# ming71/rotate-yolov3

Hardware: AMD Instinct MI355X
Metric: images/sec fwd+bwd at 608^2 (train step, backend=hip) (higher is better)
Workload: dtype bf16; 1 GPU; configs[3]: Darknet-53 train step (fwd + riou loss + bwd + grad all-reduce + SGD), bs=64/GPU 608x608, synthetic HRSC-shaped targets; global_batch=64, parallelism=dp1, gradients=250 MB fp32 in 4 flat buckets, fp32 on the wire

## Files before the change

include/ryolo.h:

```cpp
#ifndef RYOLO_H
#define RYOLO_H

#include <stddef.h>
#include <stdint.h>

#ifdef __cplusplus
extern "C" {
#endif

#define RYOLO_OK 0
#define RYOLO_EINVAL -1
#define RYOLO_ELAUNCH -2
#define RYOLO_ETOOBIG -3

#define RYOLO_RNMS_MAX_BOXES 262144

const char *ryolo_strerror(int code);
int ryolo_abi_version(void);
const char *ryolo_build_id(void);
int ryolo_set_tuning(const char *name, const char *value);

size_t ryolo_rnms_workspace_bytes(int n);
int ryolo_rnms(const float *dets, int n, int row_stride, float thr, int64_t *keep_out, int32_t *num_keep,
               void *workspace, size_t workspace_bytes, void *stream);
// ... 190 lines not shown
#define RYOLO_ARC_UBCE 2
#define RYOLO_ARC_UCE 4
size_t ryolo_yolo_loss_bitmap_bytes_arc(long long cells, int nc, int arc);
int ryolo_yolo_loss_arc(const float *p, int bs, int na, int ny, int nx, int no, int nc, const float *w, int NT,
                        const long long *b, const long long *gj, const long long *gi, const long long *cls, const float *txy,
                        const float *twh, const float *ta, const float *anchor_vec, const float *npos, float giou, float reg_w,
                        float cls_w, float cls_pw, float obj_w, float obj_pw, int iou_mode, int arc, float fl_gamma, unsigned *bitmap,
                        float *dp, float *items, void *stream);
int ryolo_yolo_loss_nhwc_arc(const void *head, int head_cstride, const float *p, int bs, int na, int ny, int nx, int no, int nc,
                             const float *w, int NT, const long long *b, const long long *gj, const long long *gi,
                             const long long *cls, const float *txy, const float *twh, const float *ta, const float *anchor_vec,
                             const float *npos, float giou, float reg_w, float cls_w, float cls_pw, float obj_w, float obj_pw,
                             int iou_mode, int arc, float fl_gamma, unsigned *bitmap, float *dp_sparse, void *head_grad,
                             int head_grad_cstride, float *items, void *stream);
int ryolo_scale_bf16_if(const float *g, void *buf, int cstride, long long npix, int C, void *stream);

int ryolo_riou_loss_pairs(const float *pbox, const float *tbox, int n, float *iou, float *grad, void *stream);

typedef struct ryolo_sgd_job {
    void *p;
    const void *g;
    void *buf;
    long long n;
    int group, first, block_begin, block_end;
} ryolo_sgd_job;
int ryolo_sgd_step(const ryolo_sgd_job *device_jobs, int njobs, int total_blocks, const float *group_hparams, int nesterov,
                   void *stream);

#ifdef __cplusplus
}
// ... 3 lines not shown
```

rotate-yolov3_amd/csrc/loss.hip:

```cpp
#include <hip/hip_runtime.h>
#include <stdint.h>

#include "../../include/ryolo.h"
#include "riou_grad.h"

namespace {

__device__ __forceinline__ float softplusf(float x) { return fmaxf(x, 0.f) + log1pf(__expf(-fabsf(x))); }
__device__ __forceinline__ float sigmoidf(float x) { return 1.f / (1.f + __expf(-x)); }
__device__ __forceinline__ float sl1(float d) { const float a = fabsf(d); return a < 1.f ? 0.5f * d * d : a - 0.5f; }
__device__ __forceinline__ float sl1_grad(float d) { return fabsf(d) < 1.f ? d : (d > 0.f ? 1.f : -1.f); }

struct Focal { float fl, f; };
__device__ __forceinline__ Focal focal_of(float L, float gamma, bool on) {
    if (!on) return Focal{L, 1.f};
    const float e = expf(-L), q = 1.000001f - e, m = powf(q, gamma);
    return Focal{L * m, m + L * gamma * (m / q) * e};
}

__device__ __forceinline__ float wave_sum(float v) {
#pragma unroll
    for (int o = 32; o > 0; o >>= 1) v += __shfl_xor(v, o);
    return v;
}
// ... 172 lines not shown
                }
            }
        }
    }
    l_obj = wave_sum(l_obj);
    l_cls = wave_sum(l_cls);
    l_reg = wave_sum(l_reg);
    if ((threadIdx.x & 63) == 0) {
        if (l_obj != 0.f) atomicAdd(q.items + 0, l_obj);
        if (l_cls != 0.f) atomicAdd(q.items + 1, l_cls);
        if (l_reg != 0.f) atomicAdd(q.items + 2, l_reg);
    }
}

typedef __attribute__((ext_vector_type(8))) __bf16 loss_bf16x8;
template <int NO>
__global__ void __launch_bounds__(256)
yolo_loss_dense_nhwc_kernel(const __bf16 *__restrict__ head, int head_cs, long long npix, int plane, int na, int no_rt, float coef,
                            float *__restrict__ dp, const unsigned *__restrict__ bitmap, __bf16 *__restrict__ hg, int hg_cs,
                            float *__restrict__ items) {
    const int no = NO ? NO : no_rt;
    const int cpr = na * no / 8;
    float acc = 0.f;
    const int lane = threadIdx.x & 63;
    const long long wave0 = (long long)blockIdx.x * 4 + (threadIdx.x >> 6), nwaves = (long long)gridDim.x * 4;
    auto one = [&](long long pix, int c8, const loss_bf16x8 &v) {
        const int a0 = c8 / no, k0 = c8 - a0 * no;
        int e1 = 5 - k0;
        if (e1 < 0) e1 += no;
        const int e2 = e1 + no;
        const uint4 raw = __builtin_bit_cast(uint4, v);
        auto logit = [&](int e) {
            const int w = e >> 1;
            unsigned d = raw.x;
            d = w == 1 ? raw.y : d;
            d = w == 2 ? raw.z : d;
            d = w == 3 ? raw.w : d;
            return __builtin_bit_cast(float, (e & 1) ? (d & 0xffff0000u) : (d << 16));
        };
        auto objectness = [&](float x) {
            const float ex = __expf(-fabsf(x));
            const float r = __builtin_amdgcn_rcpf(1.f + ex);
            acc += fmaxf(x, 0.f) + __logf(1.f + ex);
            return coef * (x >= 0.f ? r : ex * r);
        };
        float g1 = 0.f, g2 = 0.f;
        if (e1 < 8) g1 = objectness(logit(e1));
        if (e2 < 8) g2 = objectness(logit(e2));
        auto place = [&](float g, int e, unsigned (&ow)[4]) {
            const unsigned bits = (unsigned)__builtin_bit_cast(unsigned short, (__bf16)g) << ((e & 1) * 16);
#pragma unroll
            for (int w = 0; w < 4; w++) ow[w] |= (e >> 1) == w ? bits : 0u;
        };
        unsigned ow[4] = {0u, 0u, 0u, 0u};
        if (e1 < 8) place(g1, e1, ow);
        if (e2 < 8) place(g2, e2, ow);
        const long long bit0 = pix * na + a0;
        const int nspan = (k0 + 7) / no;
        unsigned hits = 0;
        for (int j = 0; j <= nspan; j++) hits |= ((bitmap[(bit0 + j) >> 5] >> ((bit0 + j) & 31)) & 1u) << j;
        if (hits) {
            const unsigned n = (unsigned)pix / (unsigned)plane;
            const long long cell0 = ((long long)n * na) * plane + ((unsigned)pix - n * (unsigned)plane);
            int j = 0, k = k0;
#pragma unroll
            for (int e = 0; e < 8; e++) {
                float o = (e == e1 ? g1 : 0.f) + (e == e2 ? g2 : 0.f);
                if ((hits >> j) & 1u) {
                    float *src = dp + (cell0 + (long long)(a0 + j) * plane) * no + k;
                    o += *src;
                    *src = 0.f;
                }
                const unsigned bits = (unsigned)__builtin_bit_cast(unsigned short, (__bf16)o);
                ow[e >> 1] = (e & 1) ? (ow[e >> 1] & 0xffffu) | (bits << 16) : (ow[e >> 1] & 0xffff0000u) | bits;
                if (++k == no) {
                    k = 0;
                    j++;
                }
            }
        }
        *(uint4 *)(hg + pix * hg_cs + c8) = uint4{ow[0], ow[1], ow[2], ow[3]};
    };
    for (long long pix = wave0; pix < npix; pix += nwaves)
        for (int chunk = lane; chunk < cpr; chunk += 64) one(pix, chunk * 8, *(const loss_bf16x8 *)(head + pix * head_cs + chunk * 8));
    __shared__ float wsum[4];
    acc = wave_sum(acc);
    if ((threadIdx.x & 63) == 0) wsum[threadIdx.x >> 6] = acc;
    __syncthreads();
    if (threadIdx.x == 0) {
        const float t = (wsum[0] + wsum[1]) + (wsum[2] + wsum[3]);
        if (t != 0.f) atomicAdd(items + 0, t * coef);
    }
}

__global__ void __launch_bounds__(256)
yolo_loss_dense_arc_kernel(const __bf16 *__restrict__ head, int head_cs, const float *__restrict__ p, long long cells, long long npix,
                           int plane, int na, int no, int nc, int focal, int unified, float gamma, float coef, float *__restrict__ dp,
                           const unsigned *__restrict__ bitmap, __bf16 *__restrict__ hg, int hg_cs, float *__restrict__ items) {
    float acc = 0.f;
    for (long long i = (long long)blockIdx.x * blockDim.x + threadIdx.x; i < cells; i += (long long)gridDim.x * blockDim.x) {
        float x[32], g[32];
        long long cell;
        long long pix = 0;
        int a = 0;
        if (head) {
            pix = i / na;
            a = (int)(i - pix * na);
// ... 52 lines not shown
__global__ void scale_bf16_if_kernel(const float *__restrict__ g, __bf16 *__restrict__ buf, int cs, long long npix, int C) {
    const float sc = g[0];
    if (sc == 1.f) return;
    const int cpr = C / 8;
    const long long total = npix * cpr;
    for (long long i = (long long)blockIdx.x * blockDim.x + threadIdx.x; i < total; i += (long long)gridDim.x * blockDim.x) {
        const long long pix = i / cpr;
        const int c8 = (int)(i - pix * cpr) * 8;
        loss_bf16x8 v = *(loss_bf16x8 *)(buf + pix * cs + c8);
#pragma unroll
        for (int e = 0; e < 8; e++) v[e] = (__bf16)((float)v[e] * sc);
        *(loss_bf16x8 *)(buf + pix * cs + c8) = v;
    }
}

struct BuildTargetsParams {
    const float *tpad;
    const unsigned char *valid;
    int NT, nheads, na;
    float iou_t, ang_t, cf;
    const float *ng[RYOLO_MAX_HEADS];
    const float *av[RYOLO_MAX_HEADS];
    float *w[RYOLO_MAX_HEADS];
    long long *idx[RYOLO_MAX_HEADS];
    float *box[RYOLO_MAX_HEADS];
    float *npos[RYOLO_MAX_HEADS];
};

__global__ void __launch_bounds__(256) build_targets_kernel(const BuildTargetsParams q) {
    const int t = blockIdx.x * blockDim.x + threadIdx.x;
// ... 153 lines not shown
                         const long long *cls, const float *txy, const float *twh, const float *ta, const float *anchor_vec,
                         const float *npos, float giou, float reg_w, float cls_w, float cls_pw, float obj_w, float obj_pw,
                         int iou_mode, unsigned *bitmap, float *dp_sparse, void *head_grad, int head_grad_cstride, float *items,
                         void *stream_) {
    return ryolo_yolo_loss_nhwc_arc(head, head_cstride, p, bs, na, ny, nx, no, nc, w, NT, b, gj, gi, cls, txy, twh, ta, anchor_vec, npos,
                                    giou, reg_w, cls_w, cls_pw, obj_w, obj_pw, iou_mode, 0, 0.f, bitmap, dp_sparse, head_grad,
                                    head_grad_cstride, items, stream_);
}

int ryolo_yolo_loss_nhwc_arc(const void *head, int head_cstride, const float *p, int bs, int na, int ny, int nx, int no, int nc,
                             const float *w, int NT, const long long *b, const long long *gj, const long long *gi,
                             const long long *cls, const float *txy, const float *twh, const float *ta, const float *anchor_vec,
                             const float *npos, float giou, float reg_w, float cls_w, float cls_pw, float obj_w, float obj_pw,
                             int iou_mode, int arc, float fl_gamma, unsigned *bitmap, float *dp_sparse, void *head_grad,
                             int head_grad_cstride, float *items, void *stream_) {
    if (!arc_ok(arc, no, nc)) return RYOLO_EINVAL;
    if (!head || !p || !w || !b || !gj || !gi || !cls || !txy || !twh || !ta || !anchor_vec || !npos || !bitmap || !dp_sparse ||
        !head_grad || !items)
        return RYOLO_EINVAL;
    if (bs <= 0 || na <= 0 || ny <= 0 || nx <= 0 || no < 6 + (nc > 1 ? nc : 0) || NT <= 0 || (iou_mode != 0 && iou_mode != 1))
        return RYOLO_EINVAL;
    const int C = na * no;
    if ((C & 7) || (head_cstride & 7) || (head_grad_cstride & 7) || head_cstride < C || head_grad_cstride < C ||
        ((uintptr_t)head & 15) || ((uintptr_t)head_grad & 15))
        return RYOLO_EINVAL;
    hipStream_t stream = (hipStream_t)stream_;
    const long long cells = (long long)bs * na * ny * nx, npix = (long long)bs * ny * nx;
    const float coef = obj_w / (float)cells;
    const int rc = launch_positives(p, dp_sparse, bs, na, ny, nx, no, nc, w, NT, b, gj, gi, cls, txy, twh, ta, anchor_vec, npos,
                                    giou, reg_w, cls_w, cls_pw, coef, obj_pw, iou_mode, bitmap, items, stream, arc, fl_gamma, 1);
    if (rc != RYOLO_OK) return rc;
    long long nb = (npix * (C / 8) + 255) / 256;
    if (nb > 2048) nb = 2048;
    if (nb < 1) nb = 1;
    if (arc != 0) {
        const int unified = (arc & RYOLO_ARC_UBCE) ? 1 : ((arc & RYOLO_ARC_UCE) ? 2 : 0);
        const float cf = unified == 1 ? coef / (float)(nc > 1 ? nc : 1) : (unified == 2 ? cls_w / (float)cells : coef);
        long long nbc = (cells + 255) / 256;
        if (nbc > 4096) nbc = 4096;
        hipLaunchKernelGGL(yolo_loss_dense_arc_kernel, dim3((unsigned)nbc), dim3(256), 0, stream, (const __bf16 *)head, head_cstride,
                           (const float *)nullptr, cells, npix, ny * nx, na, no, nc, (arc & RYOLO_ARC_FOCAL) ? 1 : 0, unified, fl_gamma,
                           cf, dp_sparse, bitmap, (__bf16 *)head_grad, head_grad_cstride, items);
        return hipGetLastError() == hipSuccess ? RYOLO_OK : RYOLO_ELAUNCH;
    }
    if (npix >= 0x7fffffffll) return RYOLO_EINVAL;
    nb = (npix + 3) / 4;
    if (nb > 8192) nb = 8192;
    if (no == 7)
        hipLaunchKernelGGL(yolo_loss_dense_nhwc_kernel<7>, dim3((unsigned)nb), dim3(256), 0, stream, (const __bf16 *)head,
                           head_cstride, npix, ny * nx, na, no, coef, dp_sparse, bitmap, (__bf16 *)head_grad, head_grad_cstride,
                           items);
    else
        hipLaunchKernelGGL(yolo_loss_dense_nhwc_kernel<0>, dim3((unsigned)nb), dim3(256), 0, stream, (const __bf16 *)head,
                           head_cstride, npix, ny * nx, na, no, coef, dp_sparse, bitmap, (__bf16 *)head_grad, head_grad_cstride,
                           items);
    return hipGetLastError() == hipSuccess ? RYOLO_OK : RYOLO_ELAUNCH;
}

int ryolo_scale_bf16_if(const float *g, void *buf, int cstride, long long npix, int C, void *stream) {
    if (!g || !buf || npix <= 0 || C <= 0 || (C & 7) || (cstride & 7) || cstride < C) return RYOLO_EINVAL;
    long long nb = (npix * (C / 8) + 255) / 256;
    if (nb > 2048) nb = 2048;
    hipLaunchKernelGGL(scale_bf16_if_kernel, dim3((unsigned)nb), dim3(256), 0, (hipStream_t)stream, g, (__bf16 *)buf, cstride, npix, C);
    return hipGetLastError() == hipSuccess ? RYOLO_OK : RYOLO_ELAUNCH;
}

int ryolo_yolo_loss(const float *p, int bs, int na, int ny, int nx, int no, int nc, const float *w, int NT,
                    const long long *b, const long long *gj, const long long *gi, const long long *cls, const float *txy,
                    const float *twh, const float *ta, const float *anchor_vec, const float *npos, float giou, float reg_w,
                    float cls_w, float cls_pw, float obj_w, float obj_pw, int iou_mode, unsigned *bitmap, float *dp,
// ... 40 lines not shown
```

rotate-yolov3_amd/model/hip_train_ops.py:

```python
import ctypes as C

import torch

from .. import _lib
from .hip_ops import ConvDesc, _check_nhwc, cpad

_vp = C.c_void_p
_P = C.POINTER(ConvDesc)
_lib.declare("ryolo_conv_stat_rows", C.c_int, [_P])
_lib.declare("ryolo_conv2d_bn_act_stats", C.c_int, [_P, _vp, _vp, _vp, _vp, _vp, _vp, _vp, _vp])
_lib.declare("ryolo_bn_finalize", C.c_int, [_vp, C.c_int, C.c_int, C.c_int, C.c_longlong, C.c_float, C.c_float, _vp, _vp, _vp,
                                            _vp, _vp, _vp, _vp, _vp, _vp])
_lib.declare("ryolo_bn_act_fwd", C.c_int, [_vp, C.c_int, _vp, _vp, C.c_int, _vp, _vp, C.c_int, _vp, C.c_int, C.c_longlong,
                                           C.c_int, _vp])
_lib.declare("ryolo_bn_act_bwd_workspace_bytes", C.c_size_t, [C.c_longlong, C.c_int])
_lib.declare("ryolo_bn_act_bwd", C.c_int, [_vp, C.c_int, _vp, C.c_int, _vp, _vp, _vp, _vp, C.c_int, _vp, _vp, C.c_int,
                                           C.c_longlong, C.c_int, _vp, _vp, _vp, _vp, C.c_size_t, _vp])
_lib.declare("ryolo_conv_packed_dgrad_bytes", C.c_size_t, [C.c_int, C.c_int, C.c_int, C.c_int])
_lib.declare("ryolo_conv_pack_weights_dgrad", C.c_int, [_vp, C.c_int, C.c_int, C.c_int, C.c_int, _vp, _vp, _vp])
_lib.declare("ryolo_conv_dgrad_tap_table", C.c_int, [C.c_int, C.c_int, _vp])
_lib.declare("ryolo_conv2d_dgrad", C.c_int, [_P, _vp, C.c_int, _vp, _vp, _vp, _vp, C.c_int, _vp])
_lib.declare("ryolo_conv2d_dgrad_bnreduce", C.c_int, [_P, _vp, C.c_int, _vp, _vp, _vp, _vp, C.c_int, _vp, C.c_int, _vp, _vp, _vp, _vp, _vp,
                                                      _vp, _vp])
_lib.declare("ryolo_bn_act_bwd_reduced", C.c_int, [_vp, C.c_int, _vp, C.c_int, _vp, _vp, _vp, _vp, C.c_int, _vp, _vp, C.c_int,
# ... 7 lines not shown


_lib.declare("ryolo_yolo_loss_bitmap_bytes", C.c_size_t, [C.c_longlong])
_lib.declare("ryolo_yolo_loss", C.c_int, [_vp, C.c_int, C.c_int, C.c_int, C.c_int, C.c_int, C.c_int, _vp, C.c_int, _vp, _vp, _vp,
                                          _vp, _vp, _vp, _vp, _vp, _vp, C.c_float, C.c_float, C.c_float, C.c_float, C.c_float,
                                          C.c_float, C.c_int, _vp, _vp, _vp, _vp])
_lib.declare("ryolo_yolo_loss_nhwc", C.c_int, [_vp, C.c_int, _vp, C.c_int, C.c_int, C.c_int, C.c_int, C.c_int, C.c_int, _vp, C.c_int, _vp,
                                               _vp, _vp, _vp, _vp, _vp, _vp, _vp, _vp, C.c_float, C.c_float, C.c_float, C.c_float,
                                               C.c_float, C.c_float, C.c_int, _vp, _vp, _vp, C.c_int, _vp, _vp])
_lib.declare("ryolo_scale_bf16_if", C.c_int, [_vp, _vp, C.c_int, C.c_longlong, C.c_int, _vp])
_lib.declare("ryolo_yolo_loss_bitmap_bytes_arc", C.c_size_t, [C.c_longlong, C.c_int, C.c_int])
_lib.declare("ryolo_yolo_loss_arc", C.c_int, [_vp] + [C.c_int] * 6 + [_vp, C.c_int] + [_vp] * 9 + [C.c_float] * 6 +
             [C.c_int, C.c_int, C.c_float] + [_vp] * 4)
_lib.declare("ryolo_yolo_loss_nhwc_arc", C.c_int, [_vp, C.c_int, _vp] + [C.c_int] * 6 + [_vp, C.c_int] + [_vp] * 9 + [C.c_float] * 6 +
             [C.c_int, C.c_int, C.c_float] + [_vp, _vp, _vp, C.c_int, _vp, _vp])
ARC_FOCAL, ARC_UBCE, ARC_UCE = 1, 2, 4


def arc_flags(arc):
    f = ARC_FOCAL if 'F' in arc else 0
    if 'default' in arc:
        return f
    if 'BCE' in arc:
        return f | ARC_UBCE
    if 'CE' in arc:
        return f | ARC_UCE
    raise ValueError("unknown arc %r" % (arc,))
_lib.declare("ryolo_riou_loss_pairs", C.c_int, [_vp, _vp, C.c_int, _vp, _vp, _vp])


# ... 312 lines not shown
    bs, na, ny, nx, no = p.shape
    w = hd['w'].contiguous()
    n = hd['npos'] if 'npos' in hd else w.sum()
    c = lambda t: t.contiguous()
    b, gj, gi, cls = c(hd['b']), c(hd['gj']), c(hd['gi']), c(hd['cls'])
    txy, twh, ta, av = c(hd['gxy']), c(hd['gwh']), c(hd['ga']), c(hd['av'].float())
    _lib.check(_lib.lib().ryolo_yolo_loss_arc(p.data_ptr(), bs, na, ny, nx, no, nc, w.data_ptr(), w.shape[1], b.data_ptr(),
                                              gj.data_ptr(), gi.data_ptr(), cls.data_ptr(), txy.data_ptr(), twh.data_ptr(),
                                              ta.data_ptr(), av.data_ptr(), n.data_ptr(), float(h['giou']), float(h['reg']),
                                              float(h['cls']), float(h['cls_pw']), float(h['obj']), float(h['obj_pw']),
                                              1 if h.get('riou', 0) else 0, int(arc), float(h.get('fl_gamma', 0.0)),
                                              bitmap.data_ptr(), dp.data_ptr(), items.data_ptr(), _s(p.device)),
               "ryolo_yolo_loss_arc")


def yolo_loss_head_nhwc(head, p, hd, nc, h, bitmap, dp_sparse, head_g, items, arc=0):
    bs, na, ny, nx, no = p.shape
    w = hd['w'].contiguous()
    n = hd['npos'] if 'npos' in hd else w.sum()
    c = lambda t: t.contiguous()
    b, gj, gi, cls = c(hd['b']), c(hd['gj']), c(hd['gi']), c(hd['cls'])
    txy, twh, ta, av = c(hd['gxy']), c(hd['gwh']), c(hd['ga']), c(hd['av'].float())
    _lib.check(_lib.lib().ryolo_yolo_loss_nhwc_arc(head.data_ptr(), head.stride(2), p.data_ptr(), bs, na, ny, nx, no, nc, w.data_ptr(),
                                                   w.shape[1], b.data_ptr(), gj.data_ptr(), gi.data_ptr(), cls.data_ptr(),
                                                   txy.data_ptr(), twh.data_ptr(), ta.data_ptr(), av.data_ptr(), n.data_ptr(),
                                                   float(h['giou']), float(h['reg']), float(h['cls']), float(h['cls_pw']),
                                                   float(h['obj']), float(h['obj_pw']), 1 if h.get('riou', 0) else 0, int(arc),
                                                   float(h.get('fl_gamma', 0.0)), bitmap.data_ptr(), dp_sparse.data_ptr(),
                                                   head_g.data_ptr(), head_g.stride(2), items.data_ptr(), _s(p.device)),
               "ryolo_yolo_loss_nhwc_arc")


def scale_bf16_if(g, buf):
    n, hh, ww, cc = buf.shape
    _lib.check(_lib.lib().ryolo_scale_bf16_if(g.data_ptr(), buf.data_ptr(), buf.stride(2), n * hh * ww, cc, _s(buf.device)),
               "ryolo_scale_bf16_if")


class RotatedIoU(torch.autograd.Function):

    @staticmethod
    def forward(ctx, pbox, tbox):
        if not pbox.is_cuda:
            raise RuntimeError("RotatedIoU runs on the HIP kernel only (got a CPU tensor)")
        p = pbox.detach().float().contiguous()
        t = tbox.detach().float().contiguous()
        n = p.shape[0]
        iou = torch.empty(n, dtype=torch.float32, device=p.device)
        grad = torch.empty(n, 5, dtype=torch.float32, device=p.device)
        _lib.check(_lib.lib().ryolo_riou_loss_pairs(p.data_ptr(), t.data_ptr(), n, iou.data_ptr(), grad.data_ptr(), _s(p.device)),
                   "ryolo_riou_loss_pairs")
# ... 43 lines not shown
```

rotate-yolov3_amd/model/loss_static.py:

```python
import math

import os

import torch
import torch.nn.functional as F

from .loss import _core


def pad_targets(targets, capacity):
    nt = int(targets.shape[0])
    if nt > capacity:
        raise ValueError("pad_targets: %d targets exceed the capacity %d" % (nt, capacity))
    tpad = torch.zeros(capacity, 7, dtype=torch.float32, device=targets.device)
    valid = torch.zeros(capacity, dtype=torch.bool, device=targets.device)
    if nt:
        tpad[:nt] = targets
        valid[:nt] = True
    return tpad, valid


def _smooth_l1(a, b):
    d = (a - b).abs()
    return torch.where(d < 1.0, 0.5 * d * d, d - 0.5)
# ... 109 lines not shown
        return fused.static_loss.clone()

    @staticmethod
    def backward(ctx, g):
        if ctx.stamp != ctx.state['stamp']:
            raise RuntimeError("fused compute_loss: backward() of a loss whose head gradients were overwritten by a later "
                               "compute_loss call on the same engine (call backward before computing the next loss)")
        if ctx.used:
            raise RuntimeError("fused compute_loss: second backward() through the same loss (the head-gradient buffers were "
                               "scaled in place by the first; retain_graph is not supported on the fused path)")
        ctx.used = True
        pg = ctx.fused.pg
        heads = ctx.fused.head_grads
        if heads is not None:
            from . import hip_train_ops as tr
            g1 = g.detach().reshape(1).float()
            for hg in heads:
                tr.scale_bf16_if(g1, hg)
        else:
            for buf in pg:
                buf.mul_(g)
        return (None,) + tuple(pg)


class FusedLoss(object):

    def __init__(self, model, capacity=512, impl='hip'):
        self.model = model
        self.impl = impl
        self.capacity = int(capacity)
        self._last_state = None

    def _engine_of(self, p):
# ... 50 lines not shown
                    eng.graph_fallback = "loss: %s: %s" % (type(e).__name__, str(e).splitlines()[0][:200] if str(e) else "")
                    import warnings
                    warnings.warn("fused loss: hipGraph capture failed (%s); continuing with eager launches" % eng.graph_fallback)
                    try:
                        torch.cuda.synchronize(dev)
                    except Exception:
                        pass
                    self._body(st)
            if st['graph'] is not None:
                st['graph'].replay()
        st['calls'] += 1
        st['stamp'] = st.get('stamp', 0) + 1
        self._last_state = st
        if st.get('head_g') is not None:
            eng.head_g_ready = True
        loss = _FusedLossFn.apply(self, *p)
        return loss, torch.cat((st['items'][:3], loss.detach()))

    def _make_state(self, eng, hyp, key):
        dev = eng.device
        if not hasattr(eng, "static_pg"):
            eng.static_pg = [torch.zeros_like(q) for q in eng.p]
        h = self.model.hyp if getattr(self.model, 'hyp', None) else hyp
        pairs = getattr(eng, 'head_pairs', None)
        nhwc = self.impl == 'hip' and pairs is not None and all(
            (hd.shape[-1] % 8 == 0 and q.shape[1] * q.shape[4] == hd.shape[-1]) for (hd, _), q in zip(pairs, eng.p))
        if nhwc:
            eng.fused_nhwc = True
            for buf in eng.static_pg:
                buf.zero_()
        return dict(key=key, hyp=dict(hyp), calls=0, graph=None, pg=eng.static_pg, eng=eng,
                    head=[a for a, _ in pairs] if nhwc else None, head_g=[b for _, b in pairs] if nhwc else None,
                    leaves=[q.detach().requires_grad_(True) for q in eng.p],
                    t=torch.zeros(self.capacity, 7, device=dev), valid=torch.zeros(self.capacity, dtype=torch.bool, device=dev),
                    loss=torch.zeros(1, device=dev), items=torch.zeros(4, device=dev),
                    pw=(torch.tensor([h['cls_pw']], dtype=torch.float32, device=dev),
                        torch.tensor([h['obj_pw']], dtype=torch.float32, device=dev)))

    def _body(self, st):
        if self.impl == 'hip':
            return self._body_hip(st)
        with torch.enable_grad():
            loss, items = compute_loss_static(st['leaves'], st['t'], st['valid'], self.model, st['hyp'], pos_weights=st['pw'])
            grads = torch.autograd.grad(loss, st['leaves'])
        with torch.no_grad():
            for buf, g in zip(st['pg'], grads):
                buf.copy_(g)
            st['loss'].copy_(loss.detach())
            st['items'].copy_(items)

    def _body_hip(self, st):
        from . import hip_train_ops as tr
        core = self.model
        h = core.hyp if getattr(core, 'hyp', None) else st['hyp']
        with torch.no_grad():
            if 'bt' not in st:
                st['bt'] = tr.BuildTargets(core, self.capacity, st['t'].device)
                st['valid_u8'] = torch.zeros(self.capacity, dtype=torch.uint8, device=st['t'].device)
            st['valid_u8'].copy_(st['valid'])
            st['bt'].run(st['t'], st['valid_u8'], h, st['hyp']['context_factor'])
            heads = st['bt'].heads()
            arc = tr.arc_flags(core.arc)
            if 'bitmaps' not in st:
                st['bitmaps'] = [tr.yolo_loss_bitmap(q, core.nc, arc) for q in st['leaves']]
            st['items'].zero_()
            for k, (q, hd, bm, dp) in enumerate(zip(st['leaves'], heads, st['bitmaps'], st['pg'])):
                bm.zero_()
                if st.get('head_g') is not None:
                    tr.yolo_loss_head_nhwc(st['head'][k], q.detach(), hd, core.nc, h, bm, dp, st['head_g'][k], st['items'], arc)
                else:
                    tr.yolo_loss_head(q.detach(), hd, core.nc, h, bm, dp, st['items'], arc)

            st['items'][3:4].copy_(st['items'][:3].sum(0, keepdim=True))
            st['loss'].copy_(st['items'][3:4])
```

rotate-yolov3_amd/model/train_engine.py:

```python
import ctypes as C
import os

import torch
import torch.nn as nn

from .. import _lib
from . import hip_ops as ops
from . import hip_train_ops as tr
from . import plan
from .engine import HipEngine


class _Fn(torch.autograd.Function):
    @staticmethod
    def forward(ctx, engine, x, anchor):
        ctx.engine = engine
        outs = engine.forward(x)
        return tuple(outs)

    @staticmethod
    def backward(ctx, *grads):
        ctx.engine.backward(grads)
        return None, None, None

# ... 71 lines not shown
            elif kind in ('add', 'up'):
                fwd.append((kind, i, tuple(tv(v) for v in rec)))
            elif kind == 'yolo':
                m = mods[i]
                c, h, w = tp.shapes[i]
                anchors = m.anchors.to(device=device, dtype=torch.float32).contiguous()
                pbuf = torch.empty((self.bs, m.na, h, w, model.nc + 6), dtype=torch.float32, device=device)
                io = None
                if model.nc + 6 > 96 or m.na * (model.nc + 6) > 1024:
                    io = torch.empty((self.bs, m.na * h * w, model.nc + 6), dtype=torch.float32, device=device)
                self.p.append(pbuf)
                fwd.append(('yolo', i, (tv(rec[0]), tv(rec[1]), m, anchors, pbuf, io, h, w)))
        self.head_pairs = [(pl[0], pl[1]) for kind, _, pl in fwd if kind == 'yolo']
        self.fused_nhwc = False
        self.head_g_ready = False
        self.batch_reduce = os.environ.get('RYOLO_WGRAD_BATCH_REDUCE', '1') != '0'
        self._wr_batches = {}
        self._ws_w_bytes = max(wgrad_ws, 256)
        self._ws_w = None
        self.ws_b = torch.empty(max(bn_ws, 256), dtype=torch.uint8, device=device)

        self.bplan = [(kind, i, pl, flags) for (kind, i, pl), (_, _, flags) in zip(reversed(fwd), tp.backward)]

    @staticmethod
    def _conv_attrs(m):
        conv = HipEngine._conv_of(m)
        other = [type(s_).__name__ for s_ in m if not isinstance(s_, (nn.Conv2d, nn.BatchNorm2d, nn.PReLU, nn.LeakyReLU))
                 and type(s_).__name__ != 'Mish']
        return dict(cout=conv.out_channels, k=conv.kernel_size[0], s=conv.stride[0], pad=conv.padding[0],
                    bn=HipEngine._bn_of(m) is not None, act=None,
# ... 248 lines not shown
                stride = float(max(self.H, self.W)) / float(max(hh, ww))
                _lib.check(L.ryolo_yolo_decode(head.data_ptr(), head.stride(2), self.bs, hh, ww, m.na, self.model.nc + 6,
                                               anchors.data_ptr(), stride, 1.0, 0, io.data_ptr() if io is not None else None, m.na * hh * ww, 0,
                                               pbuf.data_ptr(), _lib.stream_ptr(dev)), "ryolo_yolo_decode")
                if (m.nx, m.ny) != (ww, hh):
                    from .models import create_grids
                    create_grids(m, (self.H, self.W), (ww, hh), dev)

    def backward(self, pgrads):
        dev = self.device
        with torch.cuda.device(dev), torch.no_grad():
            if not hasattr(self, "static_pg"):
                self.static_pg = [torch.zeros_like(p) for p in self.p]
            ready = self.head_g_ready
            self.head_g_ready = False
            for k, (buf, g) in enumerate(zip(self.static_pg, pgrads)):
                if g is not None and ready and g.data_ptr() == buf.data_ptr():
                    continue
                if g is None:
                    buf.zero_()
                elif g.data_ptr() != buf.data_ptr():
                    buf.copy_(g)
                tr.pgrad_to_nhwc(buf, self.head_pairs[k][1])
                if self.fused_nhwc and g is not None:
                    buf.zero_()
            self._check_direct_sink()
            self._grad_of(next(self.model.parameters()))
            segs = self._segments()
            if self.batch_reduce:
                self._ensure_reduce_batches(segs)
            if self.g_bwd is None:
                self.g_bwd = [None] * len(segs)
            for k, (lo, hi, params) in enumerate(segs):
                if not self.use_graph or self.steps < 2 or self.force_eager:
                    self._backward_launch(lo, hi)
                else:
                    if self.g_bwd[k] is None:
                        self.g_bwd[k] = self._capture(lambda lo=lo, hi=hi: self._backward_launch(lo, hi))
                    if self.g_bwd[k] is not None:
                        self.g_bwd[k].replay()
                self._flush_param_grads(params)
            self.steps += 1

    def _backward_launch(self, lo=0, hi=None):
        dev = self.device
        L = _lib.lib()
        pgrads = self.static_pg
# ... 22 lines not shown
                                              self._grad_of(bn.weight), self._grad_of(bn.bias), dsl, self._grad_of(conv.weight),
                                              conv.in_channels, True, b['ws0f'])
                        return
                    elif b['recompute']:
                        if 'ws0' not in b:
                            b['ws0'] = tr.conv0_bn_bwd_ws(dev)
                        tr.conv0_bn_bwd(b['desc'], b['xin'], b['packed'], dy, b['stats'], b['actcode'], b['slope'], b['dz'],
                                        self._grad_of(bn.weight), self._grad_of(bn.bias), dsl, b['ws0'])
                    elif b.get('red_part') is not None:
                        tr.bn_act_bwd_reduced(b['z'], dy, b['stats'], 1, b['slope'], b['dz'],
                                              self._grad_of(bn.weight), self._grad_of(bn.bias), dsl, b['red_part'], self.ws_b)
                    else:
                        tr.bn_act_bwd(b['z'], dy, b['stats'], b['actcode'], b['slope'], b['dz'],
                                      self._grad_of(bn.weight), self._grad_of(bn.bias), dsl, self.ws_b)
                elif conv.bias is not None:
                    tr.bn_act_bwd(b['z'], dy, None, 0, None, None, None, self._grad_of(conv.bias), None, self.ws_b)
                if self.batch_reduce:
                    tr.conv_wgrad_partials(b['desc'], b['xin'], b['dz'], conv.in_channels, self._grad_of(conv.weight), True, b['ws_w'])
                else:
                    tr.conv_wgrad(b['desc'], b['xin'], b['dz'], conv.in_channels, self._grad_of(conv.weight), True, self.ws_w)
                if b['xin_g'] is not None:
                    y = b.get('red_for')
                    if y is not None:
                        tr.conv_dgrad_bnreduce(b['desc'], b['dz'], b['packed_d'], self.ones, self.zeros, b['xin_g'], not in_first,
                                               y['z'], y['stats'], y['slope'], y['red_part'])
                    else:
                        tr.conv_dgrad(b['desc'], b['dz'], b['packed_d'], self.ones, self.zeros, b['xin_g'], not in_first)
            elif kind == 'add':
                dyv = pl[5]
                self._passthrough(dyv, pl[3], flags[0])
                self._passthrough(dyv, pl[4], flags[1])
# ... 45 lines not shown
```

Baseline: 1341 images/s.

## Fuse head conv bias-gradient reduction into dense NHWC loss kernel

The dense NHWC YOLO loss kernel can now accumulate per-block partial column sums of the bf16 head gradient into a bias_part buffer. A small two-stage reduction kernel later folds these partials and applies the loss gradient scale to produce the head conv bias gradient, replacing a full bn_act_bwd pass over the head gradient. Separately, the per-head bf16 gradient scaling launches are batched into one multi-head kernel using a persistent device scale tensor. This adds shared-memory accumulation to the loss kernel and a separate graph cache per mode, and relies on the loss scale being linear so scaling after reduction matches.

```diff
diff --git a/include/ryolo.h b/include/ryolo.h
--- a/include/ryolo.h
+++ b/include/ryolo.h
@@ -228,6 +228,18 @@
                              int iou_mode, int arc, float fl_gamma, unsigned *bitmap, float *dp_sparse, void *head_grad,
                              int head_grad_cstride, float *items, void *stream);
 int ryolo_scale_bf16_if(const float *g, void *buf, int cstride, long long npix, int C, void *stream);
+int ryolo_scale_bf16_if_heads(const float *g, void *const *bufs, const int *cstrides, const long long *npixs, const int *Cs, int nheads,
+                              void *stream);
+
+int ryolo_yolo_loss_dbias_rows(int bs, int na, int ny, int nx, int no, int arc);
+size_t ryolo_head_dbias_part_floats(int rows, int C);
+int ryolo_yolo_loss_nhwc_dbias(const void *head, int head_cstride, const float *p, int bs, int na, int ny, int nx, int no, int nc,
+                               const float *w, int NT, const long long *b, const long long *gj, const long long *gi,
+                               const long long *cls, const float *txy, const float *twh, const float *ta, const float *anchor_vec,
+                               const float *npos, float giou, float reg_w, float cls_w, float cls_pw, float obj_w, float obj_pw,
+                               int iou_mode, int arc, float fl_gamma, unsigned *bitmap, float *dp_sparse, void *head_grad,
+                               int head_grad_cstride, float *items, float *bias_part, int bias_part_rows, void *stream);
+int ryolo_head_dbias_finalize(float *part, int rows, int C, const float *scale, float *dbias, void *stream);
 
 int ryolo_riou_loss_pairs(const float *pbox, const float *tbox, int n, float *iou, float *grad, void *stream);
 
diff --git a/rotate-yolov3_amd/csrc/loss.hip b/rotate-yolov3_amd/csrc/loss.hip
--- a/rotate-yolov3_amd/csrc/loss.hip
+++ b/rotate-yolov3_amd/csrc/loss.hip
@@ -210,14 +210,20 @@
 }
 
 typedef __attribute__((ext_vector_type(8))) __bf16 loss_bf16x8;
-template <int NO>
+template <int NO, bool DB>
 __global__ void __launch_bounds__(256)
 yolo_loss_dense_nhwc_kernel(const __bf16 *__restrict__ head, int head_cs, long long npix, int plane, int na, int no_rt, float coef,
                             float *__restrict__ dp, const unsigned *__restrict__ bitmap, __bf16 *__restrict__ hg, int hg_cs,
-                            float *__restrict__ items) {
+                            float *__restrict__ items, float *__restrict__ bias_part) {
     const int no = NO ? NO : no_rt;
     const int cpr = na * no / 8;
     float acc = 0.f;
+    float bs1 = 0.f, bs2 = 0.f;
+    __shared__ float bred[DB ? 4 : 1][DB ? 512 : 1];
+    if (DB) {
+#pragma unroll
+        for (int e = 0; e < 8; e++) bred[threadIdx.x >> 6][(threadIdx.x & 63) * 8 + e] = 0.f;
+    }
     const int lane = threadIdx.x & 63;
     const long long wave0 = (long long)blockIdx.x * 4 + (threadIdx.x >> 6), nwaves = (long long)gridDim.x * 4;
     auto one = [&](long long pix, int c8, const loss_bf16x8 &v) {
@@ -243,14 +249,15 @@
         float g1 = 0.f, g2 = 0.f;
         if (e1 < 8) g1 = objectness(logit(e1));
         if (e2 < 8) g2 = objectness(logit(e2));
-        auto place = [&](float g, int e, unsigned (&ow)[4]) {
-            const unsigned bits = (unsigned)__builtin_bit_cast(unsigned short, (__bf16)g) << ((e & 1) * 16);
+        const __bf16 b1 = (__bf16)g1, b2 = (__bf16)g2;
+        auto place = [&](__bf16 g, int e, unsigned (&ow)[4]) {
+            const unsigned bits = (unsigned)__builtin_bit_cast(unsigned short, g) << ((e & 1) * 16);
 #pragma unroll
             for (int w = 0; w < 4; w++) ow[w] |= (e >> 1) == w ? bits : 0u;
         };
         unsigned ow[4] = {0u, 0u, 0u, 0u};
-        if (e1 < 8) place(g1, e1, ow);
-        if (e2 < 8) place(g2, e2, ow);
+        if (e1 < 8) place(b1, e1, ow);
+        if (e2 < 8) place(b2, e2, ow);
         const long long bit0 = pix * na + a0;
         const int nspan = (k0 + 7) / no;
         unsigned hits = 0;
@@ -267,13 +274,18 @@
                     o += *src;
                     *src = 0.f;
                 }
-                const unsigned bits = (unsigned)__builtin_bit_cast(unsigned short, (__bf16)o);
+                const __bf16 ob = (__bf16)o;
+                if (DB) bred[threadIdx.x >> 6][c8 + e] += (float)ob;
+                const unsigned bits = (unsigned)__builtin_bit_cast(unsigned short, ob);
                 ow[e >> 1] = (e & 1) ? (ow[e >> 1] & 0xffffu) | (bits << 16) : (ow[e >> 1] & 0xffff0000u) | bits;
                 if (++k == no) {
                     k = 0;
                     j++;
                 }
             }
+        } else if (DB) {
+            bs1 += (float)b1;
+            bs2 += (float)b2;
         }
         *(uint4 *)(hg + pix * hg_cs + c8) = uint4{ow[0], ow[1], ow[2], ow[3]};
     };
@@ -287,6 +299,51 @@
         const float t = (wsum[0] + wsum[1]) + (wsum[2] + wsum[3]);
         if (t != 0.f) atomicAdd(items + 0, t * coef);
     }
+    if (DB) {
+        const int C = cpr * 8, wv = threadIdx.x >> 6;
+        if (lane < cpr) {
+            const int c8 = lane * 8, k0 = c8 % no;
+            int e1 = 5 - k0;
+            if (e1 < 0) e1 += no;
+            const int e2 = e1 + no;
+#pragma unroll
+            for (int e = 0; e < 8; e++) bred[wv][c8 + e] += (e == e1 ? bs1 : 0.f) + (e == e2 ? bs2 : 0.f);
+        }
+        __syncthreads();
+        for (int c = threadIdx.x; c < C; c += 256)
+            bias_part[(size_t)blockIdx.x * C + c] = (bred[0][c] + bred[1][c]) + (bred[2][c] + bred[3][c]);
+    }
+}
+
+constexpr int DBIAS_FOLD = 64, DBIAS_FOLD_MIN_ROWS = 512;
+__global__ void __launch_bounds__(1024)
+head_dbias_sum_kernel(const float *__restrict__ part, int nrows, int C, int per, float *__restrict__ out,
+                      const float *__restrict__ scale, float *__restrict__ dbias) {
+    __shared__ float red[32][33];
+    const int cx = threadIdx.x & 31, ry = threadIdx.x >> 5;
+    const int c = blockIdx.x * 32 + cx, g = blockIdx.y;
+    const int r0 = g * per, r1 = min(nrows, r0 + per);
+    float a = 0.f;
+    if (c < C) {
+        for (int s0 = r0 + ry; s0 < r1; s0 += 32 * 8) {
+            float v[8];
+#pragma unroll
+            for (int u = 0; u < 8; u++) {
+                const int s = s0 + 32 * u;
+                v[u] = s < r1 ? part[(size_t)s * C + c] : 0.f;
+            }
+            a += ((v[0] + v[1]) + (v[2] + v[3])) + ((v[4] + v[5]) + (v[6] + v[7]));
+        }
+    }
+    red[ry][cx] = a;
+    __syncthreads();
+    for (int h = 16; h > 0; h >>= 1) {
+        if (ry < h) red[ry][cx] += red[ry + h][cx];
+        __syncthreads();
+    }
+    if (ry != 0 || c >= C) return;
+    if (dbias) dbias[c] += red[0][cx] * scale[0];
+    else out[(size_t)g * C + c] = red[0][cx];
 }
 
 __global__ void __launch_bounds__(256)
@@ -369,6 +426,32 @@
     }
 }
 
+struct ScaleHeads {
+    __bf16 *buf[RYOLO_MAX_HEADS];
+    long long npix[RYOLO_MAX_HEADS];
+    int cs[RYOLO_MAX_HEADS], C[RYOLO_MAX_HEADS];
+};
+__global__ void scale_bf16_if_heads_kernel(const float *__restrict__ g, const ScaleHeads q) {
+    const float sc = g[0];
+    if (sc == 1.f) return;
+    __bf16 *buf = q.buf[0];
+    long long npix = q.npix[0];
+    int cs = q.cs[0], C = q.C[0];
+#pragma unroll
+    for (int h = 1; h < RYOLO_MAX_HEADS; h++)
+        if ((int)blockIdx.y == h) { buf = q.buf[h]; npix = q.npix[h]; cs = q.cs[h]; C = q.C[h]; }
+    const int cpr = C / 8;
+    const long long total = npix * cpr;
+    for (long long i = (long long)blockIdx.x * blockDim.x + threadIdx.x; i < total; i += (long long)gridDim.x * blockDim.x) {
+        const long long pix = i / cpr;
+        const int c8 = (int)(i - pix * cpr) * 8;
+        loss_bf16x8 v = *(loss_bf16x8 *)(buf + pix * cs + c8);
+#pragma unroll
+        for (int e = 0; e < 8; e++) v[e] = (__bf16)((float)v[e] * sc);
+        *(loss_bf16x8 *)(buf + pix * cs + c8) = v;
+    }
+}
+
 struct BuildTargetsParams {
     const float *tpad;
     const unsigned char *valid;
@@ -552,7 +635,31 @@
                              const float *npos, float giou, float reg_w, float cls_w, float cls_pw, float obj_w, float obj_pw,
                              int iou_mode, int arc, float fl_gamma, unsigned *bitmap, float *dp_sparse, void *head_grad,
                              int head_grad_cstride, float *items, void *stream_) {
+    return ryolo_yolo_loss_nhwc_dbias(head, head_cstride, p, bs, na, ny, nx, no, nc, w, NT, b, gj, gi, cls, txy, twh, ta, anchor_vec, npos,
+                                      giou, reg_w, cls_w, cls_pw, obj_w, obj_pw, iou_mode, arc, fl_gamma, bitmap, dp_sparse, head_grad,
+                                      head_grad_cstride, items, nullptr, 0, stream_);
+}
+
+static long long dense_nhwc_blocks(long long npix) {
+    const long long nb = (npix + 3) / 4;
+    return nb > 8192 ? 8192 : nb;
+}
+
+int ryolo_yolo_loss_dbias_rows(int bs, int na, int ny, int nx, int no, int arc) {
+    if (bs <= 0 || na <= 0 || ny <= 0 || nx <= 0 || no < 6 || arc != 0) return 0;
+    const long long C = (long long)na * no, npix = (long long)bs * ny * nx;
+    if ((C & 7) || C > 512 || npix >= 0x7fffffffll) return 0;
+    return (int)dense_nhwc_blocks(npix);
+}
+
+int ryolo_yolo_loss_nhwc_dbias(const void *head, int head_cstride, const float *p, int bs, int na, int ny, int nx, int no, int nc,
+                               const float *w, int NT, const long long *b, const long long *gj, const long long *gi,
+                               const long long *cls, const float *txy, const float *twh, const float *ta, const float *anchor_vec,
+                               const float *npos, float giou, float reg_w, float cls_w, float cls_pw, float obj_w, float obj_pw,
+                               int iou_mode, int arc, float fl_gamma, unsigned *bitmap, float *dp_sparse, void *head_grad,
+                               int head_grad_cstride, float *items, float *bias_part, int bias_part_rows, void *stream_) {
     if (!arc_ok(arc, no, nc)) return RYOLO_EINVAL;
+    if (bias_part && (bias_part_rows <= 0 || bias_part_rows != ryolo_yolo_loss_dbias_rows(bs, na, ny, nx, no, arc))) return RYOLO_EINVAL;
     if (!head || !p || !w || !b || !gj || !gi || !cls || !txy || !twh || !ta || !anchor_vec || !npos || !bitmap || !dp_sparse ||
         !head_grad || !items)
         return RYOLO_EINVAL;
@@ -582,16 +689,56 @@
         return hipGetLastError() == hipSuccess ? RYOLO_OK : RYOLO_ELAUNCH;
     }
     if (npix >= 0x7fffffffll) return RYOLO_EINVAL;
-    nb = (npix + 3) / 4;
-    if (nb > 8192) nb = 8192;
-    if (no == 7)
-        hipLaunchKernelGGL(yolo_loss_dense_nhwc_kernel<7>, dim3((unsigned)nb), dim3(256), 0, stream, (const __bf16 *)head,
-                           head_cstride, npix, ny * nx, na, no, coef, dp_sparse, bitmap, (__bf16 *)head_grad, head_grad_cstride,
-                           items);
-    else
-        hipLaunchKernelGGL(yolo_loss_dense_nhwc_kernel<0>, dim3((unsigned)nb), dim3(256), 0, stream, (const __bf16 *)head,
-                           head_cstride, npix, ny * nx, na, no, coef, dp_sparse, bitmap, (__bf16 *)head_grad, head_grad_cstride,
-                           items);
+    nb = dense_nhwc_blocks(npix);
+#define RYOLO_DENSE_NHWC(NO_, DB_)                                                                                              \
+    hipLaunchKernelGGL((yolo_loss_dense_nhwc_kernel<NO_, DB_>), dim3((unsigned)nb), dim3(256), 0, stream, (const __bf16 *)head, \
+                       head_cstride, npix, ny * nx, na, no, coef, dp_sparse, bitmap, (__bf16 *)head_grad, head_grad_cstride,    \
+                       items, bias_part)
+    if (no == 7) {
+        if (bias_part) RYOLO_DENSE_NHWC(7, true); else RYOLO_DENSE_NHWC(7, false);
+    } else {
+        if (bias_part) RYOLO_DENSE_NHWC(0, true); else RYOLO_DENSE_NHWC(0, false);
+    }
+#undef RYOLO_DENSE_NHWC
+    return hipGetLastError() == hipSuccess ? RYOLO_OK : RYOLO_ELAUNCH;
+}
+
+size_t ryolo_head_dbias_part_floats(int rows, int C) {
+    return rows <= 0 || C <= 0 ? 0 : (size_t)(rows + DBIAS_FOLD) * C;
+}
+
+int ryolo_head_dbias_finalize(float *part, int rows, int C, const float *scale, float *dbias, void *stream_) {
+    if (!part || rows <= 0 || C <= 0 || !scale || !dbias) return RYOLO_EINVAL;
+    hipStream_t stream = (hipStream_t)stream_;
+    const float *src = part;
+    int n = rows;
+    if (rows >= DBIAS_FOLD_MIN_ROWS) {
+        float *folded = part + (size_t)rows * C;
+        const int per = (rows + DBIAS_FOLD - 1) / DBIAS_FOLD;
+        hipLaunchKernelGGL(head_dbias_sum_kernel, dim3((C + 31) / 32, (rows + per - 1) / per), dim3(1024), 0, stream, src, rows, C, per,
+                           folded, (const float *)nullptr, (float *)nullptr);
+        src = folded;
+        n = (rows + per - 1) / per;
+    }
+    hipLaunchKernelGGL(head_dbias_sum_kernel, dim3((C + 31) / 32, 1), dim3(1024), 0, stream, src, n, C, n, (float *)nullptr, scale, dbias);
+    return hipGetLastError() == hipSuccess ? RYOLO_OK : RYOLO_ELAUNCH;
+}
+
+int ryolo_scale_bf16_if_heads(const float *g, void *const *bufs, const int *cstrides, const long long *npixs, const int *Cs, int nheads,
+                              void *stream) {
+    if (!g || !bufs || !cstrides || !npixs || !Cs || nheads <= 0 || nheads > RYOLO_MAX_HEADS) return RYOLO_EINVAL;
+    ScaleHeads q;
+    long long most = 0;
+    for (int h = 0; h < RYOLO_MAX_HEADS; h++) {
+        const int k = h < nheads ? h : 0;
+        if (!bufs[k] || npixs[k] <= 0 || Cs[k] <= 0 || (Cs[k] & 7) || (cstrides[k] & 7) || cstrides[k] < Cs[k]) return RYOLO_EINVAL;
+        q.buf[h] = (__bf16 *)bufs[k]; q.npix[h] = npixs[k]; q.cs[h] = cstrides[k]; q.C[h] = Cs[k];
+        const long long t = npixs[k] * (Cs[k] / 8);
+        most = t > most ? t : most;
+    }
+    long long nb = (most + 255) / 256;
+    if (nb > 2048) nb = 2048;
+    hipLaunchKernelGGL(scale_bf16_if_heads_kernel, dim3((unsigned)nb, nheads), dim3(256), 0, (hipStream_t)stream, g, q);
     return hipGetLastError() == hipSuccess ? RYOLO_OK : RYOLO_ELAUNCH;
 }
 
diff --git a/rotate-yolov3_amd/model/hip_train_ops.py b/rotate-yolov3_amd/model/hip_train_ops.py
--- a/rotate-yolov3_amd/model/hip_train_ops.py
+++ b/rotate-yolov3_amd/model/hip_train_ops.py
@@ -45,6 +45,12 @@
              [C.c_int, C.c_int, C.c_float] + [_vp] * 4)
 _lib.declare("ryolo_yolo_loss_nhwc_arc", C.c_int, [_vp, C.c_int, _vp] + [C.c_int] * 6 + [_vp, C.c_int] + [_vp] * 9 + [C.c_float] * 6 +
              [C.c_int, C.c_int, C.c_float] + [_vp, _vp, _vp, C.c_int, _vp, _vp])
+_lib.declare("ryolo_yolo_loss_nhwc_dbias", C.c_int, [_vp, C.c_int, _vp] + [C.c_int] * 6 + [_vp, C.c_int] + [_vp] * 9 + [C.c_float] * 6 +
+             [C.c_int, C.c_int, C.c_float] + [_vp, _vp, _vp, C.c_int, _vp, _vp, C.c_int, _vp])
+_lib.declare("ryolo_yolo_loss_dbias_rows", C.c_int, [C.c_int] * 6)
+_lib.declare("ryolo_head_dbias_part_floats", C.c_size_t, [C.c_int, C.c_int])
+_lib.declare("ryolo_head_dbias_finalize", C.c_int, [_vp, C.c_int, C.c_int, _vp, _vp, _vp])
+_lib.declare("ryolo_scale_bf16_if_heads", C.c_int, [_vp, _vp, _vp, _vp, _vp, C.c_int, _vp])
 ARC_FOCAL, ARC_UBCE, ARC_UCE = 1, 2, 4
 
 
@@ -387,13 +393,39 @@
                "ryolo_yolo_loss_arc")
 
 
-def yolo_loss_head_nhwc(head, p, hd, nc, h, bitmap, dp_sparse, head_g, items, arc=0):
+def head_dbias_part(p, arc=0):
+    bs, na, ny, nx, no = p.shape
+    rows = _lib.lib().ryolo_yolo_loss_dbias_rows(bs, na, ny, nx, no, int(arc))
+    if rows <= 0:
+        return None
+    part = torch.zeros(_lib.lib().ryolo_head_dbias_part_floats(rows, na * no), dtype=torch.float32, device=p.device)
+    part.rows = rows
+    return part
+
+
+def head_dbias_finalize(part, C_, scale, dbias):
+    _lib.check(_lib.lib().ryolo_head_dbias_finalize(part.data_ptr(), part.rows, C_, scale.data_ptr(), dbias.data_ptr(), _s(part.device)),
+               "ryolo_head_dbias_finalize")
+
+
+def yolo_loss_head_nhwc(head, p, hd, nc, h, bitmap, dp_sparse, head_g, items, arc=0, bias_part=None):
     bs, na, ny, nx, no = p.shape
     w = hd['w'].contiguous()
     n = hd['npos'] if 'npos' in hd else w.sum()
     c = lambda t: t.contiguous()
     b, gj, gi, cls = c(hd['b']), c(hd['gj']), c(hd['gi']), c(hd['cls'])
     txy, twh, ta, av = c(hd['gxy']), c(hd['gwh']), c(hd['ga']), c(hd['av'].float())
+    if bias_part is not None:
+        _lib.check(_lib.lib().ryolo_yolo_loss_nhwc_dbias(head.data_ptr(), head.stride(2), p.data_ptr(), bs, na, ny, nx, no, nc,
+                                                         w.data_ptr(), w.shape[1], b.data_ptr(), gj.data_ptr(), gi.data_ptr(),
+                                                         cls.data_ptr(), txy.data_ptr(), twh.data_ptr(), ta.data_ptr(), av.data_ptr(),
+                                                         n.data_ptr(), float(h['giou']), float(h['reg']), float(h['cls']),
+                                                         float(h['cls_pw']), float(h['obj']), float(h['obj_pw']),
+                                                         1 if h.get('riou', 0) else 0, int(arc), float(h.get('fl_gamma', 0.0)),
+                                                         bitmap.data_ptr(), dp_sparse.data_ptr(), head_g.data_ptr(), head_g.stride(2),
+                                                         items.data_ptr(), bias_part.data_ptr(), bias_part.rows, _s(p.device)),
+                   "ryolo_yolo_loss_nhwc_dbias")
+        return
     _lib.check(_lib.lib().ryolo_yolo_loss_nhwc_arc(head.data_ptr(), head.stride(2), p.data_ptr(), bs, na, ny, nx, no, nc, w.data_ptr(),
                                                    w.shape[1], b.data_ptr(), gj.data_ptr(), gi.data_ptr(), cls.data_ptr(),
                                                    txy.data_ptr(), twh.data_ptr(), ta.data_ptr(), av.data_ptr(), n.data_ptr(),
@@ -408,6 +440,17 @@
     n, hh, ww, cc = buf.shape
     _lib.check(_lib.lib().ryolo_scale_bf16_if(g.data_ptr(), buf.data_ptr(), buf.stride(2), n * hh * ww, cc, _s(buf.device)),
                "ryolo_scale_bf16_if")
+
+
+def scale_bf16_if_heads(g, bufs):
+    for k in range(0, len(bufs), 4):
+        bs_ = bufs[k:k + 4]
+        n = len(bs_)
+        ptrs = (C.c_void_p * n)(*[b.data_ptr() for b in bs_])
+        cs = (C.c_int * n)(*[b.stride(2) for b in bs_])
+        npix = (C.c_longlong * n)(*[b.shape[0] * b.shape[1] * b.shape[2] for b in bs_])
+        cc = (C.c_int * n)(*[b.shape[3] for b in bs_])
+        _lib.check(_lib.lib().ryolo_scale_bf16_if_heads(g.data_ptr(), ptrs, cs, npix, cc, n, _s(bs_[0].device)), "ryolo_scale_bf16_if_heads")
 
 
 class RotatedIoU(torch.autograd.Function):
diff --git a/rotate-yolov3_amd/model/loss_static.py b/rotate-yolov3_amd/model/loss_static.py
--- a/rotate-yolov3_amd/model/loss_static.py
+++ b/rotate-yolov3_amd/model/loss_static.py
@@ -147,9 +147,9 @@
         heads = ctx.fused.head_grads
         if heads is not None:
             from . import hip_train_ops as tr
-            g1 = g.detach().reshape(1).float()
-            for hg in heads:
-                tr.scale_bf16_if(g1, hg)
+            g1 = ctx.state['gscale']
+            g1.copy_(g.detach().reshape(1))
+            tr.scale_bf16_if_heads(g1, heads)
         else:
             for buf in pg:
                 buf.mul_(g)
@@ -230,6 +230,7 @@
         self._last_state = st
         if st.get('head_g') is not None:
             eng.head_g_ready = True
+            eng.head_dbias = (st['bias_part'], st['gscale']) if st.get('bias_part') is not None else None
         loss = _FusedLossFn.apply(self, *p)
         return loss, torch.cat((st['items'][:3], loss.detach()))
 
@@ -249,7 +250,7 @@
                     head=[a for a, _ in pairs] if nhwc else None, head_g=[b for _, b in pairs] if nhwc else None,
                     leaves=[q.detach().requires_grad_(True) for q in eng.p],
                     t=torch.zeros(self.capacity, 7, device=dev), valid=torch.zeros(self.capacity, dtype=torch.bool, device=dev),
-                    loss=torch.zeros(1, device=dev), items=torch.zeros(4, device=dev),
+                    loss=torch.zeros(1, device=dev), items=torch.zeros(4, device=dev), gscale=torch.ones(1, device=dev),
                     pw=(torch.tensor([h['cls_pw']], dtype=torch.float32, device=dev),
                         torch.tensor([h['obj_pw']], dtype=torch.float32, device=dev)))
 
@@ -279,11 +280,15 @@
             arc = tr.arc_flags(core.arc)
             if 'bitmaps' not in st:
                 st['bitmaps'] = [tr.yolo_loss_bitmap(q, core.nc, arc) for q in st['leaves']]
+                parts = [tr.head_dbias_part(q, arc) for q in st['leaves']] if (
+                    st.get('head_g') is not None and os.environ.get('RYOLO_HEAD_DBIAS', '1') != '0') else [None]
+                st['bias_part'] = parts if all(q is not None for q in parts) else None
             st['items'].zero_()
             for k, (q, hd, bm, dp) in enumerate(zip(st['leaves'], heads, st['bitmaps'], st['pg'])):
                 bm.zero_()
                 if st.get('head_g') is not None:
-                    tr.yolo_loss_head_nhwc(st['head'][k], q.detach(), hd, core.nc, h, bm, dp, st['head_g'][k], st['items'], arc)
+                    tr.yolo_loss_head_nhwc(st['head'][k], q.detach(), hd, core.nc, h, bm, dp, st['head_g'][k], st['items'], arc,
+                                           bias_part=st['bias_part'][k] if st['bias_part'] is not None else None)
                 else:
                     tr.yolo_loss_head(q.detach(), hd, core.nc, h, bm, dp, st['items'], arc)
 
diff --git a/rotate-yolov3_amd/model/train_engine.py b/rotate-yolov3_amd/model/train_engine.py
--- a/rotate-yolov3_amd/model/train_engine.py
+++ b/rotate-yolov3_amd/model/train_engine.py
@@ -109,6 +109,13 @@
         self.head_pairs = [(pl[0], pl[1]) for kind, _, pl in fwd if kind == 'yolo']
         self.fused_nhwc = False
         self.head_g_ready = False
+        self.head_dbias = None
+        self._dbias_fused = False
+        self._g_bwd_modes = {}
+        for k, (_, hg) in enumerate(self.head_pairs):
+            for b in self.blocks:
+                if b['bn'] is None and b['conv'].bias is not None and b['dy'].data_ptr() == hg.data_ptr() and b['dy'].shape == hg.shape:
+                    b['head_k'] = k
         self.batch_reduce = os.environ.get('RYOLO_WGRAD_BATCH_REDUCE', '1') != '0'
         self._wr_batches = {}
         self._ws_w_bytes = max(wgrad_ws, 256)
@@ -387,6 +394,8 @@
                 self.static_pg = [torch.zeros_like(p) for p in self.p]
             ready = self.head_g_ready
             self.head_g_ready = False
+            dbias_fused = bool(ready and self.head_dbias is not None and len(pgrads) == len(self.static_pg) and all(
+                g is not None and g.data_ptr() == buf.data_ptr() for buf, g in zip(self.static_pg, pgrads)))
             for k, (buf, g) in enumerate(zip(self.static_pg, pgrads)):
                 if g is not None and ready and g.data_ptr() == buf.data_ptr():
                     continue
@@ -403,7 +412,9 @@
             if self.batch_reduce:
                 self._ensure_reduce_batches(segs)
             if self.g_bwd is None:
-                self.g_bwd = [None] * len(segs)
+                self._g_bwd_modes = {}
+            self._dbias_fused = dbias_fused
+            self.g_bwd = self._g_bwd_modes.setdefault(dbias_fused, [None] * len(segs))
             for k, (lo, hi, params) in enumerate(segs):
                 if not self.use_graph or self.steps < 2 or self.force_eager:
                     self._backward_launch(lo, hi)
@@ -456,7 +467,11 @@
                         tr.bn_act_bwd(b['z'], dy, b['stats'], b['actcode'], b['slope'], b['dz'],
                                       self._grad_of(bn.weight), self._grad_of(bn.bias), dsl, self.ws_b)
                 elif conv.bias is not None:
-                    tr.bn_act_bwd(b['z'], dy, None, 0, None, None, None, self._grad_of(conv.bias), None, self.ws_b)
+                    if self._dbias_fused and b.get('head_k') is not None:
+                        parts, gscale = self.head_dbias
+                        tr.head_dbias_finalize(parts[b['head_k']], b['C'], gscale, self._grad_of(conv.bias))
+                    else:
+                        tr.bn_act_bwd(b['z'], dy, None, 0, None, None, None, self._grad_of(conv.bias), None, self.ws_b)
                 if self.batch_reduce:
                     tr.conv_wgrad_partials(b['desc'], b['xin'], b['dz'], conv.in_channels, self._grad_of(conv.weight), True, b['ws_w'])
                 else:
```

Result: no change. 1346 images/s, median of 6 (+0.3%).
